# lucidrains/audiolm-pytorch

Measured on NVIDIA H100. Metric: CoarseTransformer tokens/sec fwd+bwd seq2048, higher is better.
Workload: dtype bf16

## Files before the change

audiolm_pytorch_b200/csrc/ffn_loss_misc.cu:

```cuda
#include <stdlib.h>

#include "alm_common.cuh"

namespace alm {

constexpr int FF_THREADS = 256;
constexpr int FF_MAX_CHUNKS = 4;

__device__ __forceinline__ void unpack8b(const uint4& u, float (&f)[8]) {
  f[0] = bf16_lo(u.x); f[1] = bf16_hi(u.x); f[2] = bf16_lo(u.y); f[3] = bf16_hi(u.y);
  f[4] = bf16_lo(u.z); f[5] = bf16_hi(u.z); f[6] = bf16_lo(u.w); f[7] = bf16_hi(u.w);
}
__device__ __forceinline__ uint32_t pk2b(float a, float b) {
  __nv_bfloat162 v = __floats2bfloat162_rn(a, b);
  return *reinterpret_cast<uint32_t*>(&v);
}
__device__ __forceinline__ uint4 pack8b(const float (&f)[8]) {
  return make_uint4(pk2b(f[0], f[1]), pk2b(f[2], f[3]), pk2b(f[4], f[5]), pk2b(f[6], f[7]));
}

template <int N>
__device__ __forceinline__ void block_sum256(float (&v)[N], float* buf ) {
  const int lane = threadIdx.x & 31, warp = threadIdx.x >> 5;
#pragma unroll
  for (int i = 0; i < N; ++i) v[i] = warp_sum(v[i]);
  __syncthreads();
  if (lane == 0) {
#pragma unroll
    for (int i = 0; i < N; ++i) buf[i * 8 + warp] = v[i];
  }
  __syncthreads();
#pragma unroll
  for (int i = 0; i < N; ++i) {
    float s = 0.f;
#pragma unroll
    for (int w = 0; w < FF_THREADS / 32; ++w) s += buf[i * 8 + w];
    v[i] = s;
  }
}

template <int N, int NT>
__device__ __forceinline__ void block_sum_nt(float (&v)[N], float* buf ) {
  constexpr int NW = NT / 32;
  const int lane = threadIdx.x & 31, warp = threadIdx.x >> 5;
#pragma unroll
  for (int i = 0; i < N; ++i) v[i] = warp_sum(v[i]);
  __syncthreads();
  if (lane == 0) {
#pragma unroll
    for (int i = 0; i < N; ++i) buf[i * NW + warp] = v[i];
  }
  __syncthreads();
#pragma unroll
  for (int i = 0; i < N; ++i) {
    float s = 0.f;
#pragma unroll
    for (int w = 0; w < NW; ++w) s += buf[i * NW + w];
    v[i] = s;
  }
}

__device__ __forceinline__ uint32_t row_keep_bits8(const DropoutArgs& d, uint32_t m, uint32_t c0) {
  const uint32_t hi = (c0 >> 3) & 1u;
  const uint32_t jb = c0 & ~15u;
  uint32_t own[4], other[4];
#pragma unroll
  for (int t = 0; t < 4; ++t) {
    own[t] = dropout_word(dropout_draw(d, m, jb + 4 * hi + t), m);
    other[t] = __shfl_xor_sync(0xffffffffu, own[t], 1);
  }
  uint32_t bits = 0;
#pragma unroll
  for (int e = 0; e < 8; ++e) {
    const uint32_t w = ((uint32_t)e >> 2) == hi ? own[e & 3] : other[e & 3];
    if (dropout_pick(d, make_uint4(w, w, w, w), m, c0 + e)) bits |= 1u << e;
  }
  return bits;
}

__device__ __forceinline__ float gelu_erf(float x) { return 0.5f * x * (1.f + erff(x * 0.7071067811865476f)); }

__device__ __forceinline__ float gelu_erf_grad(float x) {
  const float cdf = 0.5f * (1.f + erff(x * 0.7071067811865476f));
  const float pdf = 0.3989422804014327f * __expf(-0.5f * x * x);
  return cdf + x * pdf;
}

template <int NCH, int NT, bool DROPOUT>
__global__ void __launch_bounds__(NT)
geglu_ln_fwd_kernel(const __nv_bfloat16* __restrict__ h, long long ldh, int gate_off,
                    const float* __restrict__ gamma, __nv_bfloat16* __restrict__ gn, long long ldg,
                    float* __restrict__ stats, int M, int inner, int inner_pad, const DropoutArgs drop) {
  __shared__ float buf[2 * (NT / 32)];
  uint4 pa[NCH], pgt[NCH];
  auto load_row = [&](int row, uint4* xa, uint4* xg) {
#pragma unroll
    for (int k = 0; k < NCH; ++k) {
      const int c0 = (threadIdx.x + k * NT) * 8;
      if (c0 < inner_pad) {
        xa[k] = *reinterpret_cast<const uint4*>(h + (size_t)row * ldh + c0);
        xg[k] = *reinterpret_cast<const uint4*>(h + (size_t)row * ldh + gate_off + c0);
      }
    }
  };
  if ((int)blockIdx.x < M) load_row(blockIdx.x, pa, pgt);
  for (int m = blockIdx.x; m < M; m += gridDim.x) {
    uint4 na[NCH], ngt[NCH];
    if (m + (int)gridDim.x < M) load_row(m + gridDim.x, na, ngt);
    if (m + 2 * (int)gridDim.x < M && (threadIdx.x & 7) == 0) {
#pragma unroll
      for (int k = 0; k < NCH; ++k) {
        const int c0 = (threadIdx.x + k * NT) * 8;
        if (c0 < inner_pad) {
          asm volatile("prefetch.global.L2 [%0];" ::"l"(h + (size_t)(m + 2 * gridDim.x) * ldh + c0));
          asm volatile("prefetch.global.L2 [%0];" ::"l"(h + (size_t)(m + 2 * gridDim.x) * ldh + gate_off + c0));
        }
      }
    }
    float g[NCH][8];
    float s12[2] = {0.f, 0.f};
#pragma unroll
    for (int k = 0; k < NCH; ++k) {
      const int c0 = (threadIdx.x + k * NT) * 8;
#pragma unroll
      for (int e = 0; e < 8; ++e) g[k][e] = 0.f;
      if (c0 < inner_pad) {
        float a[8], gt[8];
        unpack8b(pa[k], a);
        unpack8b(pgt[k], gt);
        const int nv = min(8, inner - c0);
#pragma unroll
        for (int e = 0; e < 8; ++e) {
          float cdf, xpdf;
          gelu_parts(gt[e], cdf, xpdf);
          const float v = e < nv ? gt[e] * cdf * a[e] : 0.f;
          g[k][e] = v;
          s12[0] += v;
          s12[1] = fmaf(v, v, s12[1]);
        }
      }
    }
    block_sum_nt<2, NT>(s12, buf);
    const float mean = s12[0] / inner;
    const float rstd = rsqrtf(fmaxf(s12[1] / inner - mean * mean, 0.f) + 1e-5f);
#pragma unroll
    for (int k = 0; k < NCH; ++k) {
      const int c0 = (threadIdx.x + k * NT) * 8;
      [[maybe_unused]] uint32_t keep = 0;
      if constexpr (DROPOUT) keep = row_keep_bits8(drop, m, c0);
      if (c0 < inner_pad) {
        const int nv = min(8, inner - c0);
        float gm[8] = {0.f, 0.f, 0.f, 0.f, 0.f, 0.f, 0.f, 0.f};
        if (nv == 8) {
          const float4 g0 = __ldg(reinterpret_cast<const float4*>(gamma + c0));
          const float4 g1 = __ldg(reinterpret_cast<const float4*>(gamma + c0 + 4));
          gm[0] = g0.x; gm[1] = g0.y; gm[2] = g0.z; gm[3] = g0.w; gm[4] = g1.x; gm[5] = g1.y; gm[6] = g1.z; gm[7] = g1.w;
        } else {
#pragma unroll
          for (int e = 0; e < 8; ++e)
            if (e < nv) gm[e] = __ldg(gamma + c0 + e);
        }
        float o[8];
#pragma unroll
        for (int e = 0; e < 8; ++e) o[e] = e < nv ? (g[k][e] - mean) * rstd * gm[e] : 0.f;
        if constexpr (DROPOUT) {
#pragma unroll
          for (int e = 0; e < 8; ++e) o[e] = ((keep >> e) & 1u) ? o[e] * drop.scale : 0.f;
        }
        *reinterpret_cast<uint4*>(gn + (size_t)m * ldg + c0) = pack8b(o);
      }
    }
    if (threadIdx.x == 0) {
      stats[(size_t)m * 2] = mean;
      stats[(size_t)m * 2 + 1] = rstd;
    }
#pragma unroll
    for (int k = 0; k < NCH; ++k) { pa[k] = na[k]; pgt[k] = ngt[k]; }
  }
}

template <int NCH, int NT, bool DROPOUT>
__global__ void __launch_bounds__(NT, NT == 512 ? 2 : 1)
geglu_ln_bwd_kernel(const __nv_bfloat16* __restrict__ h, long long ldh, int gate_off,
                    const float* __restrict__ gamma, const float* __restrict__ stats,
                    const __nv_bfloat16* __restrict__ dgn, long long ldg, __nv_bfloat16* __restrict__ dh,
                    float* __restrict__ g_gamma, int M, int inner, int inner_pad, const DropoutArgs drop) {
  __shared__ float buf[2 * (NT / 32)];
  float gacc[NCH][8];
#pragma unroll
  for (int k = 0; k < NCH; ++k)
#pragma unroll
    for (int e = 0; e < 8; ++e) gacc[k][e] = 0.f;
  for (int m = blockIdx.x; m < M; m += gridDim.x) {
    if (m + (int)gridDim.x < M && (threadIdx.x & 7) == 0) {
#pragma unroll
      for (int k = 0; k < NCH; ++k) {
        const int c0 = (threadIdx.x + k * NT) * 8;
        if (c0 < inner_pad) {
          asm volatile("prefetch.global.L2 [%0];" ::"l"(h + (size_t)(m + gridDim.x) * ldh + c0));
          asm volatile("prefetch.global.L2 [%0];" ::"l"(h + (size_t)(m + gridDim.x) * ldh + gate_off + c0));
          asm volatile("prefetch.global.L2 [%0];" ::"l"(dgn + (size_t)(m + gridDim.x) * ldg + c0));
        }
      }
    }
    const float mean = stats[(size_t)m * 2], rstd = stats[(size_t)m * 2 + 1];
    float a[NCH][8], gp[NCH][8], gl[NCH][8], ge[NCH][8];
    float r2[2] = {0.f, 0.f};
#pragma unroll
    for (int k = 0; k < NCH; ++k) {
      const int c0 = (threadIdx.x + k * NT) * 8;
#pragma unroll
      for (int e = 0; e < 8; ++e) { a[k][e] = gp[k][e] = gl[k][e] = ge[k][e] = 0.f; }
      [[maybe_unused]] uint32_t keep = 0;
      if constexpr (DROPOUT) keep = row_keep_bits8(drop, m, c0);
      if (c0 < inner_pad) {
        float dv[8], gt[8];
        unpack8b(*reinterpret_cast<const uint4*>(h + (size_t)m * ldh + c0), a[k]);
        unpack8b(*reinterpret_cast<const uint4*>(h + (size_t)m * ldh + gate_off + c0), gt);
        unpack8b(*reinterpret_cast<const uint4*>(dgn + (size_t)m * ldg + c0), dv);
        if constexpr (DROPOUT) {
#pragma unroll
          for (int e = 0; e < 8; ++e) dv[e] = ((keep >> e) & 1u) ? dv[e] * drop.scale : 0.f;
        }
        const int nv = min(8, inner - c0);
        float gm[8] = {0.f, 0.f, 0.f, 0.f, 0.f, 0.f, 0.f, 0.f};
        if (nv == 8) {
          const float4 g0 = __ldg(reinterpret_cast<const float4*>(gamma + c0));
          const float4 g1 = __ldg(reinterpret_cast<const float4*>(gamma + c0 + 4));
          gm[0] = g0.x; gm[1] = g0.y; gm[2] = g0.z; gm[3] = g0.w; gm[4] = g1.x; gm[5] = g1.y; gm[6] = g1.z; gm[7] = g1.w;
        } else {
#pragma unroll
          for (int e = 0; e < 8; ++e)
            if (e < nv) gm[e] = __ldg(gamma + c0 + e);
        }
#pragma unroll
        for (int e = 0; e < 8; ++e) {
          float cdf, xpdf;
          gelu_parts(gt[e], cdf, xpdf);
          const bool ok = e < nv;
          ge[k][e] = ok ? gt[e] * cdf : 0.f;
          gp[k][e] = ok ? cdf + xpdf : 0.f;
          if (!ok) { a[k][e] = 0.f; dv[e] = 0.f; }
          const float xh = (ge[k][e] * a[k][e] - mean) * rstd;
          gl[k][e] = dv[e] * gm[e];
          gacc[k][e] = fmaf(dv[e], xh, gacc[k][e]);
          r2[0] += gl[k][e];
          r2[1] = fmaf(gl[k][e], xh, r2[1]);
        }
      }
    }
    block_sum_nt<2, NT>(r2, buf);
    const float m1 = r2[0] / inner, m2 = r2[1] / inner;
#pragma unroll
    for (int k = 0; k < NCH; ++k) {
      const int c0 = (threadIdx.x + k * NT) * 8;
      if (c0 < inner_pad) {
        const int nv = min(8, inner - c0);
        float da[8], dg8[8];
#pragma unroll
        for (int e = 0; e < 8; ++e) {
          const float xh = (ge[k][e] * a[k][e] - mean) * rstd;
          const float dg = e < nv ? rstd * (gl[k][e] - m1 - xh * m2) : 0.f;
          da[e] = dg * ge[k][e];
          dg8[e] = dg * a[k][e] * gp[k][e];
        }
        *reinterpret_cast<uint4*>(dh + (size_t)m * ldh + c0) = pack8b(da);
        *reinterpret_cast<uint4*>(dh + (size_t)m * ldh + gate_off + c0) = pack8b(dg8);
      }
    }
  }
#pragma unroll
  for (int k = 0; k < NCH; ++k) {
    const int c0 = (threadIdx.x + k * NT) * 8;
#pragma unroll
    for (int e = 0; e < 8; ++e)
      if (c0 + e < inner) atomicAdd(g_gamma + c0 + e, gacc[k][e]);
  }
}



__global__ void __launch_bounds__(FF_THREADS)
ce_fwd_bwd_kernel(const float* __restrict__ logits, long long ldl, const long long* __restrict__ labels,
                  long long ignore_index, float* __restrict__ loss_rows, __nv_bfloat16* __restrict__ dlogits,
                  long long ldd, const float* __restrict__ scale_num, const float* __restrict__ scale_den, int V,
                  int Vpad) {
  __shared__ float buf[2 * 8];
  const int r = blockIdx.x;
  const float* row = logits + (size_t)r * ldl;
  const long long label = labels[r];
  const bool ignored = (label == ignore_index);
  const bool bad_label = !ignored && (label < 0 || label >= V);
  float mx[1] = {-INFINITY};
  for (int c = threadIdx.x; c < V; c += FF_THREADS) mx[0] = fmaxf(mx[0], row[c]);
  {
    float v = warp_max(mx[0]);
    __syncthreads();
    if ((threadIdx.x & 31) == 0) buf[threadIdx.x >> 5] = v;
    __syncthreads();
    float m = buf[0];
#pragma unroll
    for (int w = 1; w < FF_THREADS / 32; ++w) m = fmaxf(m, buf[w]);
    mx[0] = m;
  }
  float sm[1] = {0.f};
  for (int c = threadIdx.x; c < V; c += FF_THREADS) sm[0] += __expf(row[c] - mx[0]);
  block_sum256<1>(sm, buf);
  const float lse = mx[0] + logf(sm[0]);
  const float nan = __int_as_float(0x7fc00000);
  if (threadIdx.x == 0) loss_rows[r] = ignored ? 0.f : bad_label ? nan : (lse - row[label]);
  if (dlogits != nullptr) {
    const float sc = ignored ? 0.f : bad_label ? nan : (*scale_num) / (*scale_den);
    __nv_bfloat16* drow = dlogits + (size_t)r * ldd;
    for (int c = threadIdx.x; c < Vpad; c += FF_THREADS) {
      float g = 0.f;
      if (c < V && !ignored) g = (__expf(row[c] - lse) - (c == label ? 1.f : 0.f)) * sc;
      drow[c] = __float2bfloat16_rn(g);
    }
  }
}

__global__ void attn_delta_kernel(const __nv_bfloat16* __restrict__ o, long long ldo,
                                  const __nv_bfloat16* __restrict__ d_o, long long lddo, float* __restrict__ delta,
                                  long long dstride, float* __restrict__ dq_acc, int b, int h, int n, int D) {
  const int gw = (blockIdx.x * blockDim.x + threadIdx.x) >> 5;
  const int lane = threadIdx.x & 31;
  const int total = b * n * h;
  if (gw >= total) return;
  const int head = gw % h;
  const int tok = gw / h;
  float v = 0.f;
  for (int c = lane * 2; c < D; c += 64) {
    const uint32_t uo = *reinterpret_cast<const uint32_t*>(o + (size_t)tok * ldo + head * D + c);
    const uint32_t ud = *reinterpret_cast<const uint32_t*>(d_o + (size_t)tok * lddo + head * D + c);
    v += bf16_lo(uo) * bf16_lo(ud) + bf16_hi(uo) * bf16_hi(ud);
    if (dq_acc != nullptr)
      *reinterpret_cast<float2*>(dq_acc + ((size_t)tok * h + head) * D + c) = make_float2(0.f, 0.f);
  }
  v = warp_sum(v);
  if (lane == 0) {
    const int bi = tok / n, i = tok - bi * n;
    delta[((size_t)bi * h + head) * dstride + i] = v;
  }
}

__global__ void axpby_bf16_kernel(const __nv_bfloat16* __restrict__ x, long long ldx, float alpha,
                                  const __nv_bfloat16* __restrict__ y, long long ldy, float beta,
                                  __nv_bfloat16* __restrict__ out, long long ldout, long long rows, int cols) {
  const long long i = (long long)blockIdx.x * blockDim.x + threadIdx.x;
  const int half = cols / 2;
  if (i >= rows * half) return;
  const long long r = i / half;
  const int c = (int)(i - r * half) * 2;
  const uint32_t ux = *reinterpret_cast<const uint32_t*>(x + r * ldx + c);
  float lo = alpha * bf16_lo(ux), hi = alpha * bf16_hi(ux);
  if (y != nullptr) {
    const uint32_t uy = *reinterpret_cast<const uint32_t*>(y + r * ldy + c);
    lo += beta * bf16_lo(uy);
    hi += beta * bf16_hi(uy);
  }
  *reinterpret_cast<uint32_t*>(out + r * ldout + c) = pk2b(lo, hi);
}

// ... 145 lines not shown
}

__global__ void resid_ln_bwd_kernel(const float* __restrict__ r_new, const float* __restrict__ gamma,
                                    const float* __restrict__ stats, const float* __restrict__ dr_out,
                                    const __nv_bfloat16* __restrict__ dxn, const __nv_bfloat16* __restrict__ dextra,
                                    float* __restrict__ dr, __nv_bfloat16* __restrict__ dr_bf16,
                                    float* __restrict__ g_gamma, float out_scale, int M, int d) {
  const int row = (blockIdx.x * blockDim.x + threadIdx.x) >> 5, lane = threadIdx.x & 31;
  if (row >= M) return;
  const float mean = stats[(size_t)row * 2], rstd = stats[(size_t)row * 2 + 1];
  float s1 = 0.f, s2 = 0.f;
  for (int c = lane; c < d; c += 32) {
    const float xh = (r_new[(size_t)row * d + c] - mean) * rstd;
    const float dx = __bfloat162float(dxn[(size_t)row * d + c]);
    const float gl = dx * gamma[c];
    atomicAdd(g_gamma + c, dx * xh);
    s1 += gl;
    s2 = fmaf(gl, xh, s2);
  }
  const float m1 = warp_sum(s1) / d, m2 = warp_sum(s2) / d;
  for (int c = lane; c < d; c += 32) {
    const size_t i = (size_t)row * d + c;
    const float xh = (r_new[i] - mean) * rstd;
    const float gl = __bfloat162float(dxn[i]) * gamma[c];
    float v = rstd * (gl - m1 - xh * m2);
    if (dr_out) v += dr_out[i];
    if (dextra) v += __bfloat162float(dextra[i]);
    v *= out_scale;
    dr[i] = v;
    if (dr_bf16) dr_bf16[i] = __float2bfloat16_rn(v);
  }
}

__global__ void __launch_bounds__(256)
dropout_bf16_kernel(__nv_bfloat16* __restrict__ x, long long ld, long long M, int C, const DropoutArgs d) {
  const int ncb = (C + 15) / 16;
  const long long t = (long long)blockIdx.x * blockDim.x + threadIdx.x;
  const long long rest = t / ncb;
  const int cb = (int)(t - rest * ncb);
  const long long rb = rest >> 2;
  if (rb * 16 >= M) return;
  const uint32_t i0 = (uint32_t)(rb * 16 + 2 * (rest & 3));
  const uint32_t j0 = (uint32_t)cb * 16;
  uint4 dr[8];
#pragma unroll
  for (int e = 0; e < 8; ++e) dr[e] = dropout_draw(d, i0, j0 + e);
#pragma unroll
  for (int r = 0; r < 4; ++r) {
    const uint32_t row = i0 + (r & 1) + 8 * (r >> 1);
    if (row >= M) continue;
#pragma unroll
    for (int half = 0; half < 2; ++half) {
      const uint32_t c = j0 + 8 * half;
      if ((int)c >= C) continue;
      uint4* ptr = reinterpret_cast<uint4*>(x + (size_t)row * ld + c);
      float f[8];
      unpack8b(*ptr, f);
#pragma unroll
      for (int e = 0; e < 8; ++e) f[e] = dropout_pick(d, dr[e], row, c + e) ? f[e] * d.scale : 0.f;
      *ptr = pack8b(f);
    }
  }
}

}

using namespace alm;

extern "C" int alm_dropout_bf16(void* x, int64_t ld, int64_t M, int C, float p, uint64_t seed, uint32_t site,
                                alm_stream_t stream_) {
  cudaStream_t stream = reinterpret_cast<cudaStream_t>(stream_);
  ALM_REQUIRE(x && M >= 0 && C >= 0 && p >= 0.f && p < 1.f, ALM_ERR_ARG);
  ALM_REQUIRE(C % 8 == 0 && ld % 8 == 0 && ld >= C && (reinterpret_cast<uintptr_t>(x) & 15u) == 0, ALM_ERR_ALIGN);
  ALM_REQUIRE(M < (1ll << 32), ALM_ERR_UNSUPPORTED);
  if (M == 0 || C == 0 || p == 0.f) return ALM_OK;
  const long long threads = (M + 15) / 16 * 4 * ((C + 15) / 16);
  dropout_bf16_kernel<<<(unsigned)ceil_div(threads, 256LL), 256, 0, stream>>>(
      reinterpret_cast<__nv_bfloat16*>(x), ld, M, C, make_dropout_args(p, seed, site));
  ALM_CHECK_LAUNCH();
  ALM_LAUNCHED(1);
  return ALM_OK;
}

template <bool DROPOUT>
static void launch_geglu_ln_fwd(int nch, int grid, cudaStream_t stream, const __nv_bfloat16* hp, int64_t ldh,
                                int gate_off, const float* gamma, __nv_bfloat16* gp, int64_t ldg, float* stats, int M,
                                int inner, int inner_pad, const DropoutArgs& d) {
  if (nch <= 1) geglu_ln_fwd_kernel<1, 256, DROPOUT><<<grid, FF_THREADS, 0, stream>>>(hp, ldh, gate_off, gamma, gp, ldg, stats, M, inner, inner_pad, d);
  else if (nch == 2) geglu_ln_fwd_kernel<2, 256, DROPOUT><<<grid, FF_THREADS, 0, stream>>>(hp, ldh, gate_off, gamma, gp, ldg, stats, M, inner, inner_pad, d);
  else geglu_ln_fwd_kernel<4, 256, DROPOUT><<<grid, FF_THREADS, 0, stream>>>(hp, ldh, gate_off, gamma, gp, ldg, stats, M, inner, inner_pad, d);
}

extern "C" int alm_geglu_ln_fwd(const void* h, int64_t ldh, int gate_off, const float* gamma, void* gn, int64_t ldg,
                                float* stats, int M, int inner, int inner_pad, float dropout_p, uint64_t seed,
                                uint32_t site, alm_stream_t stream_) {
  cudaStream_t stream = reinterpret_cast<cudaStream_t>(stream_);
  ALM_REQUIRE(M > 0 && inner > 0 && inner_pad >= inner && inner_pad % 8 == 0, ALM_ERR_ARG);
  ALM_REQUIRE(dropout_p >= 0.f && dropout_p < 1.f, ALM_ERR_ARG);
  ALM_REQUIRE(ldh % 8 == 0 && ldg % 8 == 0 && gate_off % 8 == 0, ALM_ERR_ALIGN);
  const int nch = ceil_div(inner_pad / 8, FF_THREADS);
  ALM_REQUIRE(nch <= FF_MAX_CHUNKS, ALM_ERR_UNSUPPORTED);
  const int grid = min(M, num_sms() * 8);
  auto* hp = (const __nv_bfloat16*)h;
  auto* gp = (__nv_bfloat16*)gn;
  const DropoutArgs d = make_dropout_args(dropout_p, seed, site);
  if (dropout_p > 0.f) launch_geglu_ln_fwd<true>(nch, grid, stream, hp, ldh, gate_off, gamma, gp, ldg, stats, M, inner, inner_pad, d);
  else launch_geglu_ln_fwd<false>(nch, grid, stream, hp, ldh, gate_off, gamma, gp, ldg, stats, M, inner, inner_pad, d);
  ALM_CHECK_LAUNCH();
  ALM_LAUNCHED(1);
  return ALM_OK;
}

template <bool DROPOUT>
static void launch_geglu_ln_bwd(int nch, int threads, int grid, cudaStream_t stream, const __nv_bfloat16* hp,
                                int64_t ldh, int gate_off, const float* gamma, const float* stats,
                                const __nv_bfloat16* dg, int64_t ldg, __nv_bfloat16* dhp, float* g_gamma, int M,
                                int inner, int inner_pad, const DropoutArgs& d) {
  if (threads == 512) geglu_ln_bwd_kernel<1, 512, DROPOUT><<<grid, 512, 0, stream>>>(hp, ldh, gate_off, gamma, stats, dg, ldg, dhp, g_gamma, M, inner, inner_pad, d);
  else if (nch <= 1) geglu_ln_bwd_kernel<1, 256, DROPOUT><<<grid, FF_THREADS, 0, stream>>>(hp, ldh, gate_off, gamma, stats, dg, ldg, dhp, g_gamma, M, inner, inner_pad, d);
  else if (nch == 2) geglu_ln_bwd_kernel<2, 256, DROPOUT><<<grid, FF_THREADS, 0, stream>>>(hp, ldh, gate_off, gamma, stats, dg, ldg, dhp, g_gamma, M, inner, inner_pad, d);
  else geglu_ln_bwd_kernel<4, 256, DROPOUT><<<grid, FF_THREADS, 0, stream>>>(hp, ldh, gate_off, gamma, stats, dg, ldg, dhp, g_gamma, M, inner, inner_pad, d);
}

extern "C" int alm_geglu_ln_bwd(const void* h, int64_t ldh, int gate_off, const float* gamma, const float* stats,
                                const void* dgn, int64_t ldg, void* dh, float* g_gamma, int M, int inner,
                                int inner_pad, float dropout_p, uint64_t seed, uint32_t site, alm_stream_t stream_) {
  cudaStream_t stream = reinterpret_cast<cudaStream_t>(stream_);
  ALM_REQUIRE(M > 0 && inner > 0 && inner_pad >= inner && inner_pad % 8 == 0, ALM_ERR_ARG);
  ALM_REQUIRE(dropout_p >= 0.f && dropout_p < 1.f, ALM_ERR_ARG);
  ALM_REQUIRE(ldh % 8 == 0 && ldg % 8 == 0 && gate_off % 8 == 0, ALM_ERR_ALIGN);
  const int nch = ceil_div(inner_pad / 8, FF_THREADS);
  ALM_REQUIRE(nch <= FF_MAX_CHUNKS, ALM_ERR_UNSUPPORTED);
  auto* hp = (const __nv_bfloat16*)h;
  auto* dg = (const __nv_bfloat16*)dgn;
  auto* dhp = (__nv_bfloat16*)dh;
  static const int bwd_threads = getenv("ALM_GEGLU_BWD_THREADS") ? atoi(getenv("ALM_GEGLU_BWD_THREADS")) : 512;
  const int threads = bwd_threads == 512 && inner_pad > 2048 && inner_pad <= 4096 ? 512 : 256;
  const int grid = min(M, num_sms() * (threads == 512 ? 2 : 4));
  const DropoutArgs d = make_dropout_args(dropout_p, seed, site);
  if (dropout_p > 0.f) launch_geglu_ln_bwd<true>(nch, threads, grid, stream, hp, ldh, gate_off, gamma, stats, dg, ldg, dhp, g_gamma, M, inner, inner_pad, d);
  else launch_geglu_ln_bwd<false>(nch, threads, grid, stream, hp, ldh, gate_off, gamma, stats, dg, ldg, dhp, g_gamma, M, inner, inner_pad, d);
  ALM_CHECK_LAUNCH();
  ALM_LAUNCHED(1);
  return ALM_OK;
}

extern "C" int alm_ce_fwd_bwd(const float* logits, int64_t ldl, const int64_t* labels, int64_t ignore_index,
                              float* loss_rows, void* dlogits, int64_t ldd, const float* scale_num,
                              const float* scale_den, int rows, int V, int Vpad, alm_stream_t stream_) {
  cudaStream_t stream = reinterpret_cast<cudaStream_t>(stream_);
  ALM_REQUIRE(rows > 0 && V > 0 && Vpad >= V, ALM_ERR_ARG);
  ALM_REQUIRE(dlogits == nullptr || (scale_num && scale_den), ALM_ERR_ARG);
  ce_fwd_bwd_kernel<<<rows, FF_THREADS, 0, stream>>>(logits, ldl, (const long long*)labels, ignore_index,
                                                    loss_rows, (__nv_bfloat16*)dlogits, ldd, scale_num, scale_den, V,
                                                    Vpad);
  ALM_CHECK_LAUNCH();
  ALM_LAUNCHED(1);
  return ALM_OK;
}

extern "C" int alm_attn_delta_dh(const void* o, int64_t ldo, const void* d_o, int64_t lddo, float* delta,
                                 int64_t delta_stride, float* dq_acc, int b, int h, int n, int dim_head,
                                 alm_stream_t stream_) {
  cudaStream_t stream = reinterpret_cast<cudaStream_t>(stream_);
  ALM_REQUIRE(dim_head == 32 || dim_head == 64 || dim_head == 128, ALM_ERR_UNSUPPORTED);
  ALM_REQUIRE(b > 0 && h > 0 && n > 0, ALM_ERR_ARG);
  const long long warps = (long long)b * h * n;
  const int threads = 256;
  const long long blocks = ceil_div(warps * 32, (long long)threads);
  attn_delta_kernel<<<(unsigned)blocks, threads, 0, stream>>>((const __nv_bfloat16*)o, ldo,
                                                              (const __nv_bfloat16*)d_o, lddo, delta, delta_stride, dq_acc, b, h, n,
                                                              dim_head);
  ALM_CHECK_LAUNCH();
  ALM_LAUNCHED(1);
  return ALM_OK;
}

extern "C" int alm_attn_delta(const void* o, int64_t ldo, const void* d_o, int64_t lddo, float* delta,
                              int64_t delta_stride, float* dq_acc, int b, int h, int n, alm_stream_t stream_) {
  return alm_attn_delta_dh(o, ldo, d_o, lddo, delta, delta_stride, dq_acc, b, h, n, 64, stream_);
}

extern "C" int alm_axpby_bf16(const void* x, int64_t ldx, float alpha, const void* y, int64_t ldy, float beta,
                              void* out, int64_t ldout, int64_t rows, int cols, alm_stream_t stream_) {
  cudaStream_t stream = reinterpret_cast<cudaStream_t>(stream_);
  ALM_REQUIRE(rows > 0 && cols > 0 && cols % 2 == 0, ALM_ERR_ARG);
  ALM_REQUIRE(ldx % 2 == 0 && ldy % 2 == 0 && ldout % 2 == 0, ALM_ERR_ALIGN);
  const long long n = rows * (cols / 2);
  axpby_bf16_kernel<<<(unsigned)ceil_div(n, 256LL), 256, 0, stream>>>(
      (const __nv_bfloat16*)x, ldx, alpha, (const __nv_bfloat16*)y, ldy, beta, (__nv_bfloat16*)out, ldout, rows, cols);
  ALM_CHECK_LAUNCH();
  ALM_LAUNCHED(1);
  return ALM_OK;
}

extern "C" int alm_cast_pad_bf16(const float* src, int64_t lds, void* dst, int64_t ldd, int64_t rows, int cols,
                                 int cols_pad, alm_stream_t stream_) {
  cudaStream_t stream = reinterpret_cast<cudaStream_t>(stream_);
  ALM_REQUIRE(rows > 0 && cols > 0 && cols_pad >= cols, ALM_ERR_ARG);
  const long long n = rows * cols_pad;
  cast_pad_kernel<<<(unsigned)ceil_div(n, 256LL), 256, 0, stream>>>(src, lds, (__nv_bfloat16*)dst, ldd, rows, cols,
                                                                   cols_pad);
  ALM_CHECK_LAUNCH();
  ALM_LAUNCHED(1);
  return ALM_OK;
}

namespace alm {
__global__ void __launch_bounds__(256) cast_pad_multi_kernel(const long long* __restrict__ desc) {
  const long long* d = desc + 7 * (long long)blockIdx.y;
  const float* src = reinterpret_cast<const float*>(d[0]);
  __nv_bfloat16* dst = reinterpret_cast<__nv_bfloat16*>(d[1]);
  const long long rows = d[2], cols = d[3], cols_pad = d[4], lds = d[5], ldd = d[6];
  const long long pairs = cols_pad / 2;
  for (long long i = (long long)blockIdx.x * blockDim.x + threadIdx.x; i < rows * pairs;
       i += (long long)gridDim.x * blockDim.x) {
    const long long r = i / pairs, c = (i - r * pairs) * 2;
    const float a = c < cols ? src[r * lds + c] : 0.f;
    const float b = c + 1 < cols ? src[r * lds + c + 1] : 0.f;
    *reinterpret_cast<__nv_bfloat162*>(dst + r * ldd + c) = __floats2bfloat162_rn(a, b);
  }
}
}

extern "C" int alm_cast_pad_multi(const int64_t* desc_dev, int n, alm_stream_t stream_) {
  cudaStream_t stream = reinterpret_cast<cudaStream_t>(stream_);
  ALM_REQUIRE(desc_dev && n > 0 && n <= 65535, ALM_ERR_ARG);
// ... 79 lines not shown
```

Measured before the change: 727,300.

## Pipeline GEGLU-LayerNorm rows through cp.async shared-memory ring with width-sized CTAs

New measurement: 740,400, median of 6. Within noise of the previous version (+1.8%).

```diff
diff --git a/audiolm_pytorch_b200/csrc/ffn_loss_misc.cu b/audiolm_pytorch_b200/csrc/ffn_loss_misc.cu
--- a/audiolm_pytorch_b200/csrc/ffn_loss_misc.cu
+++ b/audiolm_pytorch_b200/csrc/ffn_loss_misc.cu
@@ -1,11 +1,18 @@
 #include <stdlib.h>
 
 #include "alm_common.cuh"
+#include "ptx_sm90.cuh"
 
 namespace alm {
 
 constexpr int FF_THREADS = 256;
-constexpr int FF_MAX_CHUNKS = 4;
+constexpr int FF_MAX_CHUNKS = 1024;
+constexpr int GEGLU_FWD_CPL = 4, GEGLU_FWD_DEPTH = 1, GEGLU_FWD_REGS = 80, GEGLU_FWD_REGS_DROPOUT = 128;
+constexpr int GEGLU_BWD_CPL = 1, GEGLU_BWD_DEPTH = 2, GEGLU_BWD_REGS = 56, GEGLU_BWD_REGS_DROPOUT = 80;
+constexpr int GEGLU_BWD_DROPOUT_CPL1_MAX = 65536 / GEGLU_BWD_REGS_DROPOUT / 32 * 32 * 8;
+static_assert(FF_MAX_CHUNKS / GEGLU_FWD_CPL * GEGLU_FWD_REGS_DROPOUT <= 65536, "forward CTA too large");
+static_assert(FF_MAX_CHUNKS / GEGLU_BWD_CPL * GEGLU_BWD_REGS <= 65536 && FF_MAX_CHUNKS / 2 * 128 <= 65536,
+              "backward CTA too large");
 
 __device__ __forceinline__ void unpack8b(const uint4& u, float (&f)[8]) {
   f[0] = bf16_lo(u.x); f[1] = bf16_hi(u.x); f[2] = bf16_lo(u.y); f[3] = bf16_hi(u.y);
@@ -35,27 +42,6 @@
     float s = 0.f;
 #pragma unroll
     for (int w = 0; w < FF_THREADS / 32; ++w) s += buf[i * 8 + w];
-    v[i] = s;
-  }
-}
-
-template <int N, int NT>
-__device__ __forceinline__ void block_sum_nt(float (&v)[N], float* buf ) {
-  constexpr int NW = NT / 32;
-  const int lane = threadIdx.x & 31, warp = threadIdx.x >> 5;
-#pragma unroll
-  for (int i = 0; i < N; ++i) v[i] = warp_sum(v[i]);
-  __syncthreads();
-  if (lane == 0) {
-#pragma unroll
-    for (int i = 0; i < N; ++i) buf[i * NW + warp] = v[i];
-  }
-  __syncthreads();
-#pragma unroll
-  for (int i = 0; i < N; ++i) {
-    float s = 0.f;
-#pragma unroll
-    for (int w = 0; w < NW; ++w) s += buf[i * NW + w];
     v[i] = s;
   }
 }
@@ -86,48 +72,78 @@
   return cdf + x * pdf;
 }
 
-template <int NCH, int NT, bool DROPOUT>
-__global__ void __launch_bounds__(NT)
+template <int CPL, int STAGES, int NS>
+struct RowRing {
+  uint4* base;
+  __device__ __forceinline__ const uint4* slot(int step, int s, int k) const {
+    return base + ((size_t)((step % STAGES) * NS + s) * CPL + k) * blockDim.x + threadIdx.x;
+  }
+  __device__ __forceinline__ void issue(int step, int row, int M, int inner_pad, const __nv_bfloat16* const (&src)[NS],
+                                        const long long (&ld)[NS]) const {
+    if (row < M) {
+#pragma unroll
+      for (int k = 0; k < CPL; ++k) {
+        const int c0 = (threadIdx.x + k * blockDim.x) * 8;
+        if (c0 < inner_pad) {
+#pragma unroll
+          for (int s = 0; s < NS; ++s) cp_async_16((void*)slot(step, s, k), src[s] + (size_t)row * ld[s] + c0);
+        }
+      }
+    }
+    cp_async_commit();
+  }
+};
+
+__device__ __forceinline__ float2 team_sum2(float x, float y, float2 (*red)[32], int step) {
+  x = warp_sum(x);
+  y = warp_sum(y);
+  if ((threadIdx.x & 31) == 0) red[step & 1][threadIdx.x >> 5] = make_float2(x, y);
+  __syncthreads();
+  float2 t = red[step & 1][0];
+  for (int w = 1; w < (int)(blockDim.x >> 5); ++w) {
+    t.x += red[step & 1][w].x;
+    t.y += red[step & 1][w].y;
+  }
+  return t;
+}
+
+__device__ __forceinline__ void load_gamma8(const float* __restrict__ gamma, int c0, int nv, float (&gm)[8]) {
+  if (nv == 8) {
+    const float4 g0 = __ldg(reinterpret_cast<const float4*>(gamma + c0));
+    const float4 g1 = __ldg(reinterpret_cast<const float4*>(gamma + c0 + 4));
+    gm[0] = g0.x; gm[1] = g0.y; gm[2] = g0.z; gm[3] = g0.w; gm[4] = g1.x; gm[5] = g1.y; gm[6] = g1.z; gm[7] = g1.w;
+  } else {
+#pragma unroll
+    for (int e = 0; e < 8; ++e) gm[e] = e < nv ? __ldg(gamma + c0 + e) : 0.f;
+  }
+}
+
+template <int CPL, int DEPTH, int REGS, bool DROPOUT>
+__global__ void __maxnreg__(REGS)
 geglu_ln_fwd_kernel(const __nv_bfloat16* __restrict__ h, long long ldh, int gate_off,
                     const float* __restrict__ gamma, __nv_bfloat16* __restrict__ gn, long long ldg,
                     float* __restrict__ stats, int M, int inner, int inner_pad, const DropoutArgs drop) {
-  __shared__ float buf[2 * (NT / 32)];
-  uint4 pa[NCH], pgt[NCH];
-  auto load_row = [&](int row, uint4* xa, uint4* xg) {
-#pragma unroll
-    for (int k = 0; k < NCH; ++k) {
-      const int c0 = (threadIdx.x + k * NT) * 8;
-      if (c0 < inner_pad) {
-        xa[k] = *reinterpret_cast<const uint4*>(h + (size_t)row * ldh + c0);
-        xg[k] = *reinterpret_cast<const uint4*>(h + (size_t)row * ldh + gate_off + c0);
-      }
-    }
-  };
-  if ((int)blockIdx.x < M) load_row(blockIdx.x, pa, pgt);
-  for (int m = blockIdx.x; m < M; m += gridDim.x) {
-    uint4 na[NCH], ngt[NCH];
-    if (m + (int)gridDim.x < M) load_row(m + gridDim.x, na, ngt);
-    if (m + 2 * (int)gridDim.x < M && (threadIdx.x & 7) == 0) {
-#pragma unroll
-      for (int k = 0; k < NCH; ++k) {
-        const int c0 = (threadIdx.x + k * NT) * 8;
-        if (c0 < inner_pad) {
-          asm volatile("prefetch.global.L2 [%0];" ::"l"(h + (size_t)(m + 2 * gridDim.x) * ldh + c0));
-          asm volatile("prefetch.global.L2 [%0];" ::"l"(h + (size_t)(m + 2 * gridDim.x) * ldh + gate_off + c0));
-        }
-      }
-    }
-    float g[NCH][8];
-    float s12[2] = {0.f, 0.f};
-#pragma unroll
-    for (int k = 0; k < NCH; ++k) {
-      const int c0 = (threadIdx.x + k * NT) * 8;
+  extern __shared__ uint4 ring_smem[];
+  __shared__ float2 red[2][32];
+  const RowRing<CPL, DEPTH + 1, 2> ring{ring_smem};
+  const __nv_bfloat16* const src[2] = {h, h + gate_off};
+  const long long ld[2] = {ldh, ldh};
+#pragma unroll
+  for (int i = 0; i < DEPTH; ++i) ring.issue(i, blockIdx.x + i * gridDim.x, M, inner_pad, src, ld);
+  for (int i = 0, m = blockIdx.x; m < M; ++i, m += gridDim.x) {
+    ring.issue(i + DEPTH, m + DEPTH * gridDim.x, M, inner_pad, src, ld);
+    cp_async_wait<DEPTH>();
+    float g[CPL][8];
+    float s1 = 0.f, s2 = 0.f;
+#pragma unroll
+    for (int k = 0; k < CPL; ++k) {
+      const int c0 = (threadIdx.x + k * blockDim.x) * 8;
 #pragma unroll
       for (int e = 0; e < 8; ++e) g[k][e] = 0.f;
       if (c0 < inner_pad) {
         float a[8], gt[8];
-        unpack8b(pa[k], a);
-        unpack8b(pgt[k], gt);
+        unpack8b(*ring.slot(i, 0, k), a);
+        unpack8b(*ring.slot(i, 1, k), gt);
         const int nv = min(8, inner - c0);
 #pragma unroll
         for (int e = 0; e < 8; ++e) {
@@ -135,32 +151,23 @@
           gelu_parts(gt[e], cdf, xpdf);
           const float v = e < nv ? gt[e] * cdf * a[e] : 0.f;
           g[k][e] = v;
-          s12[0] += v;
-          s12[1] = fmaf(v, v, s12[1]);
+          s1 += v;
+          s2 = fmaf(v, v, s2);
         }
       }
     }
-    block_sum_nt<2, NT>(s12, buf);
-    const float mean = s12[0] / inner;
-    const float rstd = rsqrtf(fmaxf(s12[1] / inner - mean * mean, 0.f) + 1e-5f);
-#pragma unroll
-    for (int k = 0; k < NCH; ++k) {
-      const int c0 = (threadIdx.x + k * NT) * 8;
+    const float2 s12 = team_sum2(s1, s2, red, i);
+    const float mean = s12.x / inner;
+    const float rstd = rsqrtf(fmaxf(s12.y / inner - mean * mean, 0.f) + 1e-5f);
+#pragma unroll
+    for (int k = 0; k < CPL; ++k) {
+      const int c0 = (threadIdx.x + k * blockDim.x) * 8;
       [[maybe_unused]] uint32_t keep = 0;
       if constexpr (DROPOUT) keep = row_keep_bits8(drop, m, c0);
       if (c0 < inner_pad) {
         const int nv = min(8, inner - c0);
-        float gm[8] = {0.f, 0.f, 0.f, 0.f, 0.f, 0.f, 0.f, 0.f};
-        if (nv == 8) {
-          const float4 g0 = __ldg(reinterpret_cast<const float4*>(gamma + c0));
-          const float4 g1 = __ldg(reinterpret_cast<const float4*>(gamma + c0 + 4));
-          gm[0] = g0.x; gm[1] = g0.y; gm[2] = g0.z; gm[3] = g0.w; gm[4] = g1.x; gm[5] = g1.y; gm[6] = g1.z; gm[7] = g1.w;
-        } else {
-#pragma unroll
-          for (int e = 0; e < 8; ++e)
-            if (e < nv) gm[e] = __ldg(gamma + c0 + e);
-        }
-        float o[8];
+        float gm[8], o[8];
+        load_gamma8(gamma, c0, nv, gm);
 #pragma unroll
         for (int e = 0; e < 8; ++e) o[e] = e < nv ? (g[k][e] - mean) * rstd * gm[e] : 0.f;
         if constexpr (DROPOUT) {
@@ -174,65 +181,57 @@
       stats[(size_t)m * 2] = mean;
       stats[(size_t)m * 2 + 1] = rstd;
     }
-#pragma unroll
-    for (int k = 0; k < NCH; ++k) { pa[k] = na[k]; pgt[k] = ngt[k]; }
-  }
-}
-
-template <int NCH, int NT, bool DROPOUT>
-__global__ void __launch_bounds__(NT, NT == 512 ? 2 : 1)
+  }
+}
+
+template <int CPL, int DEPTH, int REGS, bool DROPOUT>
+__global__ void __maxnreg__(REGS)
 geglu_ln_bwd_kernel(const __nv_bfloat16* __restrict__ h, long long ldh, int gate_off,
                     const float* __restrict__ gamma, const float* __restrict__ stats,
                     const __nv_bfloat16* __restrict__ dgn, long long ldg, __nv_bfloat16* __restrict__ dh,
                     float* __restrict__ g_gamma, int M, int inner, int inner_pad, const DropoutArgs drop) {
-  __shared__ float buf[2 * (NT / 32)];
-  float gacc[NCH][8];
-#pragma unroll
-  for (int k = 0; k < NCH; ++k)
+  extern __shared__ uint4 ring_smem[];
+  __shared__ float2 red[2][32];
+  const RowRing<CPL, DEPTH + 1, 3> ring{ring_smem};
+  const __nv_bfloat16* const src[3] = {h, h + gate_off, dgn};
+  const long long ld[3] = {ldh, ldh, ldg};
+  float gacc[CPL][8];
+#pragma unroll
+  for (int k = 0; k < CPL; ++k)
 #pragma unroll
     for (int e = 0; e < 8; ++e) gacc[k][e] = 0.f;
-  for (int m = blockIdx.x; m < M; m += gridDim.x) {
-    if (m + (int)gridDim.x < M && (threadIdx.x & 7) == 0) {
-#pragma unroll
-      for (int k = 0; k < NCH; ++k) {
-        const int c0 = (threadIdx.x + k * NT) * 8;
-        if (c0 < inner_pad) {
-          asm volatile("prefetch.global.L2 [%0];" ::"l"(h + (size_t)(m + gridDim.x) * ldh + c0));
-          asm volatile("prefetch.global.L2 [%0];" ::"l"(h + (size_t)(m + gridDim.x) * ldh + gate_off + c0));
-          asm volatile("prefetch.global.L2 [%0];" ::"l"(dgn + (size_t)(m + gridDim.x) * ldg + c0));
-        }
-      }
-    }
-    const float mean = stats[(size_t)m * 2], rstd = stats[(size_t)m * 2 + 1];
-    float a[NCH][8], gp[NCH][8], gl[NCH][8], ge[NCH][8];
-    float r2[2] = {0.f, 0.f};
-#pragma unroll
-    for (int k = 0; k < NCH; ++k) {
-      const int c0 = (threadIdx.x + k * NT) * 8;
-#pragma unroll
-      for (int e = 0; e < 8; ++e) { a[k][e] = gp[k][e] = gl[k][e] = ge[k][e] = 0.f; }
+#pragma unroll
+  for (int i = 0; i < DEPTH; ++i) ring.issue(i, blockIdx.x + i * gridDim.x, M, inner_pad, src, ld);
+  float mean = 0.f, rstd = 0.f;
+  if ((int)blockIdx.x < M) { mean = stats[(size_t)blockIdx.x * 2]; rstd = stats[(size_t)blockIdx.x * 2 + 1]; }
+  for (int i = 0, m = blockIdx.x; m < M; ++i, m += gridDim.x) {
+    ring.issue(i + DEPTH, m + DEPTH * gridDim.x, M, inner_pad, src, ld);
+    float next_mean = 0.f, next_rstd = 0.f;
+    if (m + (int)gridDim.x < M) {
+      next_mean = stats[(size_t)(m + gridDim.x) * 2];
+      next_rstd = stats[(size_t)(m + gridDim.x) * 2 + 1];
+    }
+    cp_async_wait<DEPTH>();
+    float gp[CPL][8], gl[CPL][8], ge[CPL][8];
+    float r1 = 0.f, r2 = 0.f;
+#pragma unroll
+    for (int k = 0; k < CPL; ++k) {
+      const int c0 = (threadIdx.x + k * blockDim.x) * 8;
+#pragma unroll
+      for (int e = 0; e < 8; ++e) { gp[k][e] = gl[k][e] = ge[k][e] = 0.f; }
       [[maybe_unused]] uint32_t keep = 0;
       if constexpr (DROPOUT) keep = row_keep_bits8(drop, m, c0);
       if (c0 < inner_pad) {
-        float dv[8], gt[8];
-        unpack8b(*reinterpret_cast<const uint4*>(h + (size_t)m * ldh + c0), a[k]);
-        unpack8b(*reinterpret_cast<const uint4*>(h + (size_t)m * ldh + gate_off + c0), gt);
-        unpack8b(*reinterpret_cast<const uint4*>(dgn + (size_t)m * ldg + c0), dv);
+        float a[8], dv[8], gt[8], gm[8];
+        unpack8b(*ring.slot(i, 0, k), a);
+        unpack8b(*ring.slot(i, 1, k), gt);
+        unpack8b(*ring.slot(i, 2, k), dv);
         if constexpr (DROPOUT) {
 #pragma unroll
           for (int e = 0; e < 8; ++e) dv[e] = ((keep >> e) & 1u) ? dv[e] * drop.scale : 0.f;
         }
         const int nv = min(8, inner - c0);
-        float gm[8] = {0.f, 0.f, 0.f, 0.f, 0.f, 0.f, 0.f, 0.f};
-        if (nv == 8) {
-          const float4 g0 = __ldg(reinterpret_cast<const float4*>(gamma + c0));
-          const float4 g1 = __ldg(reinterpret_cast<const float4*>(gamma + c0 + 4));
-          gm[0] = g0.x; gm[1] = g0.y; gm[2] = g0.z; gm[3] = g0.w; gm[4] = g1.x; gm[5] = g1.y; gm[6] = g1.z; gm[7] = g1.w;
-        } else {
-#pragma unroll
-          for (int e = 0; e < 8; ++e)
-            if (e < nv) gm[e] = __ldg(gamma + c0 + e);
-        }
+        load_gamma8(gamma, c0, nv, gm);
 #pragma unroll
         for (int e = 0; e < 8; ++e) {
           float cdf, xpdf;
@@ -240,45 +239,53 @@
           const bool ok = e < nv;
           ge[k][e] = ok ? gt[e] * cdf : 0.f;
           gp[k][e] = ok ? cdf + xpdf : 0.f;
-          if (!ok) { a[k][e] = 0.f; dv[e] = 0.f; }
-          const float xh = (ge[k][e] * a[k][e] - mean) * rstd;
+          if (!ok) { a[e] = 0.f; dv[e] = 0.f; }
+          const float xh = (ge[k][e] * a[e] - mean) * rstd;
           gl[k][e] = dv[e] * gm[e];
           gacc[k][e] = fmaf(dv[e], xh, gacc[k][e]);
-          r2[0] += gl[k][e];
-          r2[1] = fmaf(gl[k][e], xh, r2[1]);
+          r1 += gl[k][e];
+          r2 = fmaf(gl[k][e], xh, r2);
         }
       }
     }
-    block_sum_nt<2, NT>(r2, buf);
-    const float m1 = r2[0] / inner, m2 = r2[1] / inner;
-#pragma unroll
-    for (int k = 0; k < NCH; ++k) {
-      const int c0 = (threadIdx.x + k * NT) * 8;
+    const float2 r12 = team_sum2(r1, r2, red, i);
+    const float m1 = r12.x / inner, m2 = r12.y / inner;
+#pragma unroll
+    for (int k = 0; k < CPL; ++k) {
+      const int c0 = (threadIdx.x + k * blockDim.x) * 8;
       if (c0 < inner_pad) {
         const int nv = min(8, inner - c0);
-        float da[8], dg8[8];
+        float a[8], da[8], dg8[8];
+        unpack8b(*ring.slot(i, 0, k), a);
 #pragma unroll
         for (int e = 0; e < 8; ++e) {
-          const float xh = (ge[k][e] * a[k][e] - mean) * rstd;
+          if (e >= nv) a[e] = 0.f;
+          const float xh = (ge[k][e] * a[e] - mean) * rstd;
           const float dg = e < nv ? rstd * (gl[k][e] - m1 - xh * m2) : 0.f;
           da[e] = dg * ge[k][e];
-          dg8[e] = dg * a[k][e] * gp[k][e];
+          dg8[e] = dg * a[e] * gp[k][e];
         }
         *reinterpret_cast<uint4*>(dh + (size_t)m * ldh + c0) = pack8b(da);
         *reinterpret_cast<uint4*>(dh + (size_t)m * ldh + gate_off + c0) = pack8b(dg8);
       }
     }
-  }
-#pragma unroll
-  for (int k = 0; k < NCH; ++k) {
-    const int c0 = (threadIdx.x + k * NT) * 8;
-#pragma unroll
-    for (int e = 0; e < 8; ++e)
-      if (c0 + e < inner) atomicAdd(g_gamma + c0 + e, gacc[k][e]);
-  }
-}
-
-
+    mean = next_mean;
+    rstd = next_rstd;
+  }
+  const bool vec = (reinterpret_cast<uintptr_t>(g_gamma) & 15u) == 0;
+#pragma unroll
+  for (int k = 0; k < CPL; ++k) {
+    const int c0 = (threadIdx.x + k * blockDim.x) * 8;
+    if (vec && c0 + 8 <= inner) {
+      atomicAdd(reinterpret_cast<float4*>(g_gamma + c0), make_float4(gacc[k][0], gacc[k][1], gacc[k][2], gacc[k][3]));
+      atomicAdd(reinterpret_cast<float4*>(g_gamma + c0 + 4), make_float4(gacc[k][4], gacc[k][5], gacc[k][6], gacc[k][7]));
+    } else {
+#pragma unroll
+      for (int e = 0; e < 8; ++e)
+        if (c0 + e < inner) atomicAdd(g_gamma + c0 + e, gacc[k][e]);
+    }
+  }
+}
 
 __global__ void __launch_bounds__(FF_THREADS)
 ce_fwd_bwd_kernel(const float* __restrict__ logits, long long ldl, const long long* __restrict__ labels,
@@ -590,13 +597,26 @@
   return ALM_OK;
 }
 
-template <bool DROPOUT>
-static void launch_geglu_ln_fwd(int nch, int grid, cudaStream_t stream, const __nv_bfloat16* hp, int64_t ldh,
-                                int gate_off, const float* gamma, __nv_bfloat16* gp, int64_t ldg, float* stats, int M,
-                                int inner, int inner_pad, const DropoutArgs& d) {
-  if (nch <= 1) geglu_ln_fwd_kernel<1, 256, DROPOUT><<<grid, FF_THREADS, 0, stream>>>(hp, ldh, gate_off, gamma, gp, ldg, stats, M, inner, inner_pad, d);
-  else if (nch == 2) geglu_ln_fwd_kernel<2, 256, DROPOUT><<<grid, FF_THREADS, 0, stream>>>(hp, ldh, gate_off, gamma, gp, ldg, stats, M, inner, inner_pad, d);
-  else geglu_ln_fwd_kernel<4, 256, DROPOUT><<<grid, FF_THREADS, 0, stream>>>(hp, ldh, gate_off, gamma, gp, ldg, stats, M, inner, inner_pad, d);
+template <int CPL, int STAGES, int NS, auto kernel, typename... Args>
+static int launch_geglu(int M, int inner_pad, cudaStream_t stream, Args... args) {
+  constexpr int MAX_WARPS = FF_MAX_CHUNKS / CPL / 32;
+  const int warps = ceil_div(ceil_div(inner_pad / 8, CPL), 32);
+  const int threads = 32 * warps;
+  const size_t smem = (size_t)STAGES * NS * CPL * threads * sizeof(uint4);
+  static int resident[MAX_WARPS + 1];
+  if (resident[warps] == 0) {
+    ALM_CUDA_OK(cudaFuncSetAttribute(kernel, cudaFuncAttributeMaxDynamicSharedMemorySize,
+                                     STAGES * NS * FF_MAX_CHUNKS * (int)sizeof(uint4)));
+    int n = 0;
+    ALM_CUDA_OK(cudaOccupancyMaxActiveBlocksPerMultiprocessor(&n, kernel, threads, smem));
+    ALM_REQUIRE(n > 0, ALM_ERR_UNSUPPORTED);
+    resident[warps] = n;
+  }
+  const int grid = min(M, resident[warps] * num_sms());
+  kernel<<<grid, threads, smem, stream>>>(args...);
+  ALM_CHECK_LAUNCH();
+  ALM_LAUNCHED(1);
+  return ALM_OK;
 }
 
 extern "C" int alm_geglu_ln_fwd(const void* h, int64_t ldh, int gate_off, const float* gamma, void* gn, int64_t ldg,
@@ -606,28 +626,17 @@
   ALM_REQUIRE(M > 0 && inner > 0 && inner_pad >= inner && inner_pad % 8 == 0, ALM_ERR_ARG);
   ALM_REQUIRE(dropout_p >= 0.f && dropout_p < 1.f, ALM_ERR_ARG);
   ALM_REQUIRE(ldh % 8 == 0 && ldg % 8 == 0 && gate_off % 8 == 0, ALM_ERR_ALIGN);
-  const int nch = ceil_div(inner_pad / 8, FF_THREADS);
-  ALM_REQUIRE(nch <= FF_MAX_CHUNKS, ALM_ERR_UNSUPPORTED);
-  const int grid = min(M, num_sms() * 8);
+  ALM_REQUIRE(inner_pad / 8 <= FF_MAX_CHUNKS, ALM_ERR_UNSUPPORTED);
   auto* hp = (const __nv_bfloat16*)h;
   auto* gp = (__nv_bfloat16*)gn;
   const DropoutArgs d = make_dropout_args(dropout_p, seed, site);
-  if (dropout_p > 0.f) launch_geglu_ln_fwd<true>(nch, grid, stream, hp, ldh, gate_off, gamma, gp, ldg, stats, M, inner, inner_pad, d);
-  else launch_geglu_ln_fwd<false>(nch, grid, stream, hp, ldh, gate_off, gamma, gp, ldg, stats, M, inner, inner_pad, d);
-  ALM_CHECK_LAUNCH();
-  ALM_LAUNCHED(1);
-  return ALM_OK;
-}
-
-template <bool DROPOUT>
-static void launch_geglu_ln_bwd(int nch, int threads, int grid, cudaStream_t stream, const __nv_bfloat16* hp,
-                                int64_t ldh, int gate_off, const float* gamma, const float* stats,
-                                const __nv_bfloat16* dg, int64_t ldg, __nv_bfloat16* dhp, float* g_gamma, int M,
-                                int inner, int inner_pad, const DropoutArgs& d) {
-  if (threads == 512) geglu_ln_bwd_kernel<1, 512, DROPOUT><<<grid, 512, 0, stream>>>(hp, ldh, gate_off, gamma, stats, dg, ldg, dhp, g_gamma, M, inner, inner_pad, d);
-  else if (nch <= 1) geglu_ln_bwd_kernel<1, 256, DROPOUT><<<grid, FF_THREADS, 0, stream>>>(hp, ldh, gate_off, gamma, stats, dg, ldg, dhp, g_gamma, M, inner, inner_pad, d);
-  else if (nch == 2) geglu_ln_bwd_kernel<2, 256, DROPOUT><<<grid, FF_THREADS, 0, stream>>>(hp, ldh, gate_off, gamma, stats, dg, ldg, dhp, g_gamma, M, inner, inner_pad, d);
-  else geglu_ln_bwd_kernel<4, 256, DROPOUT><<<grid, FF_THREADS, 0, stream>>>(hp, ldh, gate_off, gamma, stats, dg, ldg, dhp, g_gamma, M, inner, inner_pad, d);
+  if (dropout_p > 0.f)
+    return launch_geglu<GEGLU_FWD_CPL, GEGLU_FWD_DEPTH + 1, 2,
+                        geglu_ln_fwd_kernel<GEGLU_FWD_CPL, GEGLU_FWD_DEPTH, GEGLU_FWD_REGS_DROPOUT, true>>(
+        M, inner_pad, stream, hp, (long long)ldh, gate_off, gamma, gp, (long long)ldg, stats, M, inner, inner_pad, d);
+  return launch_geglu<GEGLU_FWD_CPL, GEGLU_FWD_DEPTH + 1, 2,
+                      geglu_ln_fwd_kernel<GEGLU_FWD_CPL, GEGLU_FWD_DEPTH, GEGLU_FWD_REGS, false>>(
+      M, inner_pad, stream, hp, (long long)ldh, gate_off, gamma, gp, (long long)ldg, stats, M, inner, inner_pad, d);
 }
 
 extern "C" int alm_geglu_ln_bwd(const void* h, int64_t ldh, int gate_off, const float* gamma, const float* stats,
@@ -637,20 +646,24 @@
   ALM_REQUIRE(M > 0 && inner > 0 && inner_pad >= inner && inner_pad % 8 == 0, ALM_ERR_ARG);
   ALM_REQUIRE(dropout_p >= 0.f && dropout_p < 1.f, ALM_ERR_ARG);
   ALM_REQUIRE(ldh % 8 == 0 && ldg % 8 == 0 && gate_off % 8 == 0, ALM_ERR_ALIGN);
-  const int nch = ceil_div(inner_pad / 8, FF_THREADS);
-  ALM_REQUIRE(nch <= FF_MAX_CHUNKS, ALM_ERR_UNSUPPORTED);
+  ALM_REQUIRE(inner_pad / 8 <= FF_MAX_CHUNKS, ALM_ERR_UNSUPPORTED);
   auto* hp = (const __nv_bfloat16*)h;
   auto* dg = (const __nv_bfloat16*)dgn;
   auto* dhp = (__nv_bfloat16*)dh;
-  static const int bwd_threads = getenv("ALM_GEGLU_BWD_THREADS") ? atoi(getenv("ALM_GEGLU_BWD_THREADS")) : 512;
-  const int threads = bwd_threads == 512 && inner_pad > 2048 && inner_pad <= 4096 ? 512 : 256;
-  const int grid = min(M, num_sms() * (threads == 512 ? 2 : 4));
   const DropoutArgs d = make_dropout_args(dropout_p, seed, site);
-  if (dropout_p > 0.f) launch_geglu_ln_bwd<true>(nch, threads, grid, stream, hp, ldh, gate_off, gamma, stats, dg, ldg, dhp, g_gamma, M, inner, inner_pad, d);
-  else launch_geglu_ln_bwd<false>(nch, threads, grid, stream, hp, ldh, gate_off, gamma, stats, dg, ldg, dhp, g_gamma, M, inner, inner_pad, d);
-  ALM_CHECK_LAUNCH();
-  ALM_LAUNCHED(1);
-  return ALM_OK;
+  if (dropout_p > 0.f && inner_pad <= GEGLU_BWD_DROPOUT_CPL1_MAX)
+    return launch_geglu<GEGLU_BWD_CPL, GEGLU_BWD_DEPTH + 1, 3,
+                        geglu_ln_bwd_kernel<GEGLU_BWD_CPL, GEGLU_BWD_DEPTH, GEGLU_BWD_REGS_DROPOUT, true>>(
+        M, inner_pad, stream, hp, (long long)ldh, gate_off, gamma, stats, dg, (long long)ldg, dhp, g_gamma, M, inner,
+        inner_pad, d);
+  if (dropout_p > 0.f)
+    return launch_geglu<2, GEGLU_BWD_DEPTH + 1, 3, geglu_ln_bwd_kernel<2, GEGLU_BWD_DEPTH, 128, true>>(
+        M, inner_pad, stream, hp, (long long)ldh, gate_off, gamma, stats, dg, (long long)ldg, dhp, g_gamma, M, inner,
+        inner_pad, d);
+  return launch_geglu<GEGLU_BWD_CPL, GEGLU_BWD_DEPTH + 1, 3,
+                      geglu_ln_bwd_kernel<GEGLU_BWD_CPL, GEGLU_BWD_DEPTH, GEGLU_BWD_REGS, false>>(
+      M, inner_pad, stream, hp, (long long)ldh, gate_off, gamma, stats, dg, (long long)ldg, dhp, g_gamma, M, inner,
+      inner_pad, d);
 }
 
 extern "C" int alm_ce_fwd_bwd(const float* logits, int64_t ldl, const int64_t* labels, int64_t ignore_index,
```
